# zouyunkai/MedicalSemSeg

Measured on AMD Instinct MI355X. Metric: 96^3 vols/sec fwd+bwd (train), higher is better.
Workload: dtype bf16; 1 GPU; UNet base (MONAI BasicUNet 32-32-64-128-256-32) 1->3cls, 96^3 patches, DiceCE + AdamW, per-GPU batch 2; global_batch=2, parallelism=dp1, grad_sync=none (single rank)

## Files before the change

medicalsemseg_amd/csrc/channel_reduce.h:

```cpp
#pragma once
#include "common.h"

template <typename T> struct ChunkV {
    static constexpr int EPC = DT<T>::EPC;
    float v[EPC];
    MSSEG_DEVFN void load(const T* p) { Chunk<T>::load(p, v); }
    MSSEG_DEVFN void store(T* p) const { Chunk<T>::store(p, v); }
};

static inline bool vec_ok(const void* p, long long ld, int C, int esz) {
    const int epc = 16 / esz;
    return (C % epc) == 0 && (ld % epc) == 0 && (((uintptr_t)p) & 15) == 0;
}

struct RowMap {
    int groups;
    int rows_par;
};
static inline RowMap row_map(int C, int width, int nthr = 256) {
    RowMap m;
    m.groups = ceil_div(C, width);
    if (m.groups > nthr) m.groups = nthr;
    m.rows_par = nthr / m.groups;
    if (m.rows_par < 1) m.rows_par = 1;
    return m;
}

static inline long long reduce_blocks(long long S, int rows_par, int N, int C, int nper) {
    long long blocks = ceil_div_ll(S, (long long)rows_par * 8);
    long long cap = (long long)msseg_num_cus() / (N > 0 ? N : 1);
    if (cap < 1) cap = 1;
    const long long fit = (long long)(((size_t)16 << 20) / ((size_t)N * C * nper * 4));
    if (cap > fit) cap = fit;
    if (blocks > cap) blocks = cap;
    if (blocks < 1) blocks = 1;
    return blocks;
}

constexpr int RED_THREADS = 512;
constexpr int RED_STAGE2 = 16;

template <int W>
MSSEG_DEVFN void block_rows_reduce(float* red, int groups, int rows_par, int g, int rl, bool act) {
    if (act && rl < RED_STAGE2 && rl < rows_par) {
#pragma unroll
        for (int e = 0; e < W; ++e) {
            float a = 0.f, b = 0.f;
            for (int k = rl; k < rows_par; k += RED_STAGE2) {
                a += red[((k * groups + g) * W + e) * 2 + 0];
                b += red[((k * groups + g) * W + e) * 2 + 1];
            }
            red[((rl * groups + g) * W + e) * 2 + 0] = a;
            red[((rl * groups + g) * W + e) * 2 + 1] = b;
        }
    }
    __syncthreads();
}

struct FinalizeArgs {
    const float* ws; int N, nblk, C, nper, mode; float* out; float* dp0; float* dp1; int accumulate;
};
int msseg_channels_finalize_launch(const FinalizeArgs& a, hipStream_t st);
```

medicalsemseg_amd/csrc/head_conv.hip:

```cpp
#include "channel_reduce.h"

namespace {

struct HeadBwdParams {
    const void* dy; long long lddy;
    const float* w;
    const void* x; long long ldx;
    const float* stats; const float* gamma; const float* beta;
    void* da; long long ldda;
    long long S; int C, Cout; float eps, slope;
    int groups, rows_par; long long rows_per_block;
    float* ws;
    int want_dw;
};

struct HeadFinArgs {
    const float* ws; int N, nblk, C, nper, Cout; float* red; float* dbeta; float* dgamma; float* dw; int acc_norm, acc_dw;
};
__global__ __launch_bounds__(256) void head_finalize_kernel(const HeadFinArgs a) {
    __shared__ __attribute__((aligned(16))) float fin[256 * 4 + 64 * 6];
    __shared__ float tot_n[64 * 6];
    const int L = a.C * a.nper;
    for (int o = threadIdx.x; o < L; o += 256) tot_n[o] = 0.f;
    for (int n = 0; n < a.N; ++n) {
        block_rows_sum<256>(a.ws + (long long)n * a.nblk * L, a.nblk, L, fin);
        const float* t = fin + 256 * 4;
        for (int o = threadIdx.x; o < L; o += 256) {
            const int c = o / a.nper, k = o % a.nper;
            if (k < 2) a.red[((long long)n * a.C + c) * 2 + k] = t[o];
            tot_n[o] += t[o];
        }
        __syncthreads();
    }
    for (int o = threadIdx.x; o < L; o += 256) {
        const int c = o / a.nper, k = o % a.nper;
        const float tot = tot_n[o];
        if (k == 0) { if (a.dbeta) a.dbeta[c] = a.acc_norm ? a.dbeta[c] + tot : tot; }
        else if (k == 1) { if (a.dgamma) a.dgamma[c] = a.acc_norm ? a.dgamma[c] + tot : tot; }
        else if (k - 2 < a.Cout && a.dw) a.dw[(k - 2) * a.C + c] = a.acc_dw ? a.dw[(k - 2) * a.C + c] + tot : tot;
    }
}

template <typename T, bool DW>
__global__ __launch_bounds__(RED_THREADS) void head_dgrad_inbwd_kernel(const HeadBwdParams p) {
    constexpr int WD = DT<T>::EPC;
    __shared__ float red[RED_THREADS * 2 * WD];
    const int n = blockIdx.y;
    const int g = threadIdx.x % p.groups, rl = threadIdx.x / p.groups;
    const long long r0 = (long long)blockIdx.x * p.rows_per_block;
    long long r1 = r0 + p.rows_per_block;
    if (r1 > p.S) r1 = p.S;
    const T* xn = (const T*)p.x + (long long)n * p.S * p.ldx;
    const T* dyn = (const T*)p.dy + (long long)n * p.S * p.lddy;
    T* dan = (T*)p.da + (long long)n * p.S * p.ldda;
    for (int gbase = 0; gbase * WD < p.C; gbase += p.groups) {
        const int gg = gbase + g;
        const bool act = gg * WD < p.C;
        float mean[WD], rstd[WD], sc[WD], sh[WD], a0[WD], a1[WD], wv[4][WD];
        float gw[DW ? 4 : 1][WD];
#pragma unroll
        for (int e = 0; e < WD; ++e) {
            const int c = act ? gg * WD + e : 0;
            mean_rstd(p.stats, n, p.C, c, p.S, p.eps, mean[e], rstd[e]);
            sc[e] = rstd[e] * (p.gamma ? p.gamma[c] : 1.f);
            sh[e] = (p.beta ? p.beta[c] : 0.f) - mean[e] * sc[e];
            a0[e] = a1[e] = 0.f;
#pragma unroll
            for (int k = 0; k < 4; ++k) wv[k][e] = k < p.Cout ? (float)(T)p.w[k * p.C + c] : 0.f;
#pragma unroll
            for (int k = 0; k < (DW ? 4 : 1); ++k) gw[k][e] = 0.f;
        }
        if (act && rl < p.rows_par) {
            constexpr int UNR = DW ? 2 : 4;
#pragma unroll UNR
            for (long long r = r0 + rl; r < r1; r += p.rows_par) {
                ChunkV<T> xc, dc, o;
                xc.load(xn + r * p.ldx + gg * WD);
                dc.load(dyn + r * p.lddy);
#pragma unroll
                for (int e = 0; e < WD; ++e) {
                    const float da = head_da<T, WD>(dc.v, wv, e);
                    o.v[e] = da;
                    const float z = xc.v[e] * sc[e] + sh[e];
                    const float dz = z > 0.f ? da : da * p.slope;
                    a0[e] += dz;
                    a1[e] += dz * ((xc.v[e] - mean[e]) * rstd[e]);
                    if constexpr (DW) {
                        const float av = (float)(T)(z > 0.f ? z : z * p.slope);
#pragma unroll
                        for (int k = 0; k < 4; ++k) gw[k][e] += dc.v[k] * av;
                    }
                }
                if (!DW || p.da != nullptr) o.store(dan + r * p.ldda + gg * WD);
            }
        }
        constexpr int NPER = DW ? 6 : 2;
        float* wsb = p.ws + ((long long)n * gridDim.x + blockIdx.x) * p.C * NPER;
#pragma unroll
        for (int round = 0; round < NPER / 2; ++round) {
            __syncthreads();
#pragma unroll
            for (int e = 0; e < WD; ++e) {
                float v0, v1;
                if (round == 0) { v0 = a0[e]; v1 = a1[e]; }
                else { v0 = gw[DW ? 2 * round - 2 : 0][e]; v1 = gw[DW ? 2 * round - 1 : 0][e]; }
                red[(threadIdx.x * WD + e) * 2 + 0] = v0;
                red[(threadIdx.x * WD + e) * 2 + 1] = v1;
            }
            __syncthreads();
            block_rows_reduce<WD>(red, p.groups, p.rows_par, g, rl, act);
            if (act && rl == 0) {
                const int kmax = p.rows_par < RED_STAGE2 ? p.rows_par : RED_STAGE2;
#pragma unroll
                for (int e = 0; e < WD; ++e) {
                    float a = 0.f, b = 0.f;
                    for (int k = 0; k < kmax; ++k) {
                        a += red[((k * p.groups + g) * WD + e) * 2 + 0];
                        b += red[((k * p.groups + g) * WD + e) * 2 + 1];
                    }
                    wsb[(gg * WD + e) * NPER + 2 * round + 0] = a;
                    wsb[(gg * WD + e) * NPER + 2 * round + 1] = b;
                }
            }
        }
    }
}

template <typename T, int COUT>
__global__ __launch_bounds__(256) void conv1x1_head_kernel(const T* __restrict__ x, long long ldx, const float* __restrict__ w,
                                                           const float* __restrict__ bias, T* __restrict__ y, long long ldy,
                                                           long long NV, int Cin) {
    constexpr int WD = DT<T>::EPC;
    __shared__ float wS[COUT * 64];
    for (int i = threadIdx.x; i < COUT * Cin; i += 256) wS[i] = (float)(T)w[i];
    __syncthreads();
    float b[COUT];
#pragma unroll
    for (int c = 0; c < COUT; ++c) b[c] = bias ? bias[c] : 0.f;
    for (long long v = blockIdx.x * 256LL + threadIdx.x; v < NV; v += (long long)gridDim.x * 256) {
        float acc[COUT];
#pragma unroll
        for (int c = 0; c < COUT; ++c) acc[c] = b[c];
        const T* xr = x + v * ldx;
        for (int k0 = 0; k0 < Cin; k0 += 4 * WD) {
            ChunkV<T> xc[4];
#pragma unroll
            for (int j = 0; j < 4; ++j)
                if (k0 + j * WD < Cin) xc[j].load(xr + k0 + j * WD);
#pragma unroll
            for (int j = 0; j < 4; ++j)
                if (k0 + j * WD < Cin) {
#pragma unroll
                    for (int c = 0; c < COUT; ++c)
#pragma unroll
                        for (int e = 0; e < WD; ++e) acc[c] += xc[j].v[e] * wS[c * Cin + k0 + j * WD + e];
                }
        }
        T* yr = y + v * ldy;
#pragma unroll
        for (int c = 0; c < COUT; ++c) DT<T>::st(yr + c, acc[c]);
    }
}

template <typename T, int COUT>
__global__ __launch_bounds__(256) void conv1x1_head_norm_kernel(const T* __restrict__ x, long long ldx,
                                                                const float* __restrict__ stats,
                                                                const float* __restrict__ gamma, const float* __restrict__ beta,
                                                                float slope, float eps, const float* __restrict__ w,
                                                                const float* __restrict__ bias, T* __restrict__ y,
                                                                long long ldy, long long S, int Cin) {
    constexpr int WD = DT<T>::EPC;
    __shared__ float wS[COUT * 64];
    __shared__ float scS[64], shS[64];
    const int n = blockIdx.y;
    for (int i = threadIdx.x; i < COUT * Cin; i += 256) wS[i] = (float)(T)w[i];
    for (int c = threadIdx.x; c < Cin; c += 256) {
        float mean, rstd;
        mean_rstd(stats, n, Cin, c, S, eps, mean, rstd);
        const float sc = rstd * (gamma ? gamma[c] : 1.f);
        scS[c] = sc;
        shS[c] = (beta ? beta[c] : 0.f) - mean * sc;
    }
    __syncthreads();
    float b[COUT];
#pragma unroll
    for (int c = 0; c < COUT; ++c) b[c] = bias ? bias[c] : 0.f;
    const T* xn = x + (long long)n * S * ldx;
    T* yn = y + (long long)n * S * ldy;
    for (long long v = blockIdx.x * 256LL + threadIdx.x; v < S; v += (long long)gridDim.x * 256) {
        float acc[COUT];
#pragma unroll
        for (int c = 0; c < COUT; ++c) acc[c] = b[c];
        const T* xr = xn + v * ldx;
        for (int k0 = 0; k0 < Cin; k0 += 4 * WD) {
            ChunkV<T> xc[4];
#pragma unroll
            for (int j = 0; j < 4; ++j)
                if (k0 + j * WD < Cin) xc[j].load(xr + k0 + j * WD);
#pragma unroll
            for (int j = 0; j < 4; ++j)
                if (k0 + j * WD < Cin) {
#pragma unroll
                    for (int e = 0; e < WD; ++e) {
                        const int k = k0 + j * WD + e;
                        const float z = xc[j].v[e] * scS[k] + shS[k];
                        const float a = (float)(T)(z > 0.f ? z : z * slope);
#pragma unroll
                        for (int c = 0; c < COUT; ++c) acc[c] += a * wS[c * Cin + k];
                    }
                }
        }
        T* yr = yn + v * ldy;
#pragma unroll
        for (int c = 0; c < COUT; ++c) DT<T>::st(yr + c, acc[c]);
    }
}

}

extern "C" {

int msseg_conv3d_k1_head_fwd(const void* x, long long ldx, const float* w, const float* bias, void* y, long long ldy,
                             long long NV, int Cin, int Cout, int dtype, msseg_stream_t stream) {
    if (!x || !w || !y || NV < 1) MSSEG_FAIL(MSSEG_EINVAL, "conv3d_k1_head: bad args");
    const int esz = dtype == MSSEG_F32 ? 4 : 2;
    if (dtype != MSSEG_F32 && dtype != MSSEG_BF16) MSSEG_FAIL(MSSEG_EINVAL, "conv3d_k1_head: bad dtype");
    if (Cout < 1 || Cout > 4 || Cin < 1 || Cin > 64 || !vec_ok(x, ldx, Cin, esz) || ldy < Cout)
        MSSEG_FAIL(MSSEG_EINVAL, "conv3d_k1_head: needs 1 <= Cout <= 4, Cin <= 64 in 16-byte chunks (got %d -> %d)", Cin, Cout);
    const int g = stream_grid(NV);
#define HEAD(T_, C_) hipLaunchKernelGGL((conv1x1_head_kernel<T_, C_>), dim3(g), dim3(256), 0, (hipStream_t)stream, \
                                        (const T_*)x, ldx, w, bias, (T_*)y, ldy, NV, Cin)
#define HEAD_C(T_) do { if (Cout == 1) HEAD(T_, 1); else if (Cout == 2) HEAD(T_, 2); else if (Cout == 3) HEAD(T_, 3); else HEAD(T_, 4); } while (0)
    for_dtype(dtype, [&](auto t) { HEAD_C(typename decltype(t)::type); });
#undef HEAD_C
#undef HEAD
    MSSEG_CHECK_LAUNCH("conv3d_k1_head");
    return MSSEG_OK;
}

int msseg_conv3d_k1_head_bwd_fused(const void* dy, long long lddy, const float* w, void* da, long long ldda, int N,
                                   long long S, int C, int Cout, const void* yraw, long long ldyraw, const float* fwd_stats,
                                   const float* gamma, const float* beta, float slope, float eps, float* red, float* dgamma,
                                   float* dbeta, int accumulate, float* dw, int dw_accumulate, void* scratch,
                                   size_t scratch_bytes, int dtype, msseg_stream_t stream) {
    if (!dy || !w || (!da && !dw) || !yraw || !fwd_stats || !red || N < 1 || S < 1)
        MSSEG_FAIL(MSSEG_EINVAL, "conv3d_k1_head_bwd_fused: bad args");
    if (dtype != MSSEG_F32 && dtype != MSSEG_BF16) MSSEG_FAIL(MSSEG_EINVAL, "conv3d_k1_head_bwd_fused: bad dtype");
    if (int rc = scratch_ok(scratch, scratch_bytes, "conv3d_k1_head_bwd_fused")) return rc;
    const int esz = dtype == MSSEG_F32 ? 4 : 2, epc = 16 / esz;
    if (Cout < 1 || Cout > 4 || C < 1 || C > 64 || !vec_ok(yraw, ldyraw, C, esz) || (da && !vec_ok(da, ldda, C, esz)) ||
        (lddy % epc) || ((uintptr_t)dy & 15))
        MSSEG_FAIL(MSSEG_EINVAL, "conv3d_k1_head_bwd_fused: needs <= 4 classes in 16-byte aligned gradient rows and "
                                 "16-byte channel chunks (C=%d, Cout=%d, lddy=%lld)", C, Cout, lddy);
    HeadBwdParams p{dy, lddy, w, yraw, ldyraw, fwd_stats, gamma, beta, da, ldda, S, C, Cout, eps, slope, 0, 0, 0, nullptr, 0};
    p.ws = (float*)((unsigned char*)scratch + MSSEG_SCRATCH_HEADER_BYTES);
    p.want_dw = dw != nullptr;
    const int nper = dw ? 6 : 2;
    const RowMap m = row_map(C, epc, RED_THREADS);
    p.groups = m.groups; p.rows_par = m.rows_par;
    long long blocks = reduce_blocks(S, m.rows_par, N, C, nper);
    p.rows_per_block = ceil_div_ll(S, blocks);
    blocks = ceil_div_ll(S, p.rows_per_block);
    dim3 grid((unsigned)blocks, N);
    if (dw) {
        for_dtype(dtype, [&](auto t) {
            hipLaunchKernelGGL((head_dgrad_inbwd_kernel<typename decltype(t)::type, true>), grid, dim3(RED_THREADS), 0,
                               (hipStream_t)stream, p);
        });
    } else {
        for_dtype(dtype, [&](auto t) {
            hipLaunchKernelGGL((head_dgrad_inbwd_kernel<typename decltype(t)::type, false>), grid, dim3(RED_THREADS), 0,
                               (hipStream_t)stream, p);
        });
    }
    MSSEG_CHECK_LAUNCH("conv3d_k1_head_dgrad_inbwd");
    HeadFinArgs a{p.ws, N, (int)blocks, C, nper, Cout, red, dbeta, dgamma, dw, accumulate, dw_accumulate};
    hipLaunchKernelGGL(head_finalize_kernel, dim3(1), dim3(256), 0, (hipStream_t)stream, a);
    MSSEG_CHECK_LAUNCH("head_finalize");
    return MSSEG_OK;
}

int msseg_conv3d_k1_head_norm_fwd(const void* x, long long ldx, const float* stats, const float* gamma, const float* beta,
                                  float slope, float eps, const float* w, const float* bias, void* y, long long ldy, int N,
                                  long long S, int Cin, int Cout, int dtype, msseg_stream_t stream) {
    if (!x || !stats || !w || !y || N < 1 || S < 1) MSSEG_FAIL(MSSEG_EINVAL, "conv3d_k1_head_norm: bad args");
    const int esz = dtype == MSSEG_F32 ? 4 : 2;
    if (dtype != MSSEG_F32 && dtype != MSSEG_BF16) MSSEG_FAIL(MSSEG_EINVAL, "conv3d_k1_head_norm: bad dtype");
    if ((gamma == nullptr) != (beta == nullptr)) MSSEG_FAIL(MSSEG_EINVAL, "conv3d_k1_head_norm: gamma/beta go together");
    if (Cout < 1 || Cout > 4 || Cin < 1 || Cin > 64 || !vec_ok(x, ldx, Cin, esz) || ldy < Cout)
        MSSEG_FAIL(MSSEG_EINVAL, "conv3d_k1_head_norm: needs 1 <= Cout <= 4, Cin <= 64 in 16-byte chunks (got %d -> %d)", Cin, Cout);
    long long gx = ceil_div_ll(S, 256);
    const long long cap = (long long)msseg_num_cus() * 16 / N + 1;
    if (gx > cap) gx = cap;
    dim3 grid((unsigned)gx, N);
#define HEADN(T_, C_) hipLaunchKernelGGL((conv1x1_head_norm_kernel<T_, C_>), grid, dim3(256), 0, (hipStream_t)stream, \
                                         (const T_*)x, ldx, stats, gamma, beta, slope, eps, w, bias, (T_*)y, ldy, S, Cin)
#define HEADN_C(T_) do { if (Cout == 1) HEADN(T_, 1); else if (Cout == 2) HEADN(T_, 2); else if (Cout == 3) HEADN(T_, 3); else HEADN(T_, 4); } while (0)
    for_dtype(dtype, [&](auto t) { HEADN_C(typename decltype(t)::type); });
#undef HEADN_C
#undef HEADN
    MSSEG_CHECK_LAUNCH("conv3d_k1_head_norm");
    return MSSEG_OK;
}

}
```

Before: 578.4 vol/s.

## Software-pipeline head backward dW kernel loads and fuse block reduction rounds

```diff
diff --git a/medicalsemseg_amd/csrc/channel_reduce.h b/medicalsemseg_amd/csrc/channel_reduce.h
--- a/medicalsemseg_amd/csrc/channel_reduce.h
+++ b/medicalsemseg_amd/csrc/channel_reduce.h
@@ -57,6 +57,26 @@
     __syncthreads();
 }
 
+template <int NT>
+MSSEG_DEVFN void block_cols_reduce(float* red, int ncols, int rows_par, float* out, int out_cols) {
+    const int slots = rows_par < RED_STAGE2 ? rows_par : RED_STAGE2;
+    for (int item = threadIdx.x; item < slots * ncols; item += NT) {
+        const int s = item / ncols, col = item - s * ncols;
+        float a = 0.f;
+#pragma unroll 8
+        for (int k = s; k < rows_par; k += RED_STAGE2) a += red[k * ncols + col];
+        red[item] = a;
+    }
+    __syncthreads();
+    for (int col = threadIdx.x; col < out_cols; col += NT) {
+        float a = 0.f;
+#pragma unroll
+        for (int k = 0; k < RED_STAGE2; ++k)
+            if (k < slots) a += red[k * ncols + col];
+        out[col] = a;
+    }
+}
+
 struct FinalizeArgs {
     const float* ws; int N, nblk, C, nper, mode; float* out; float* dp0; float* dp1; int accumulate;
 };
diff --git a/medicalsemseg_amd/csrc/head_bwd.h b/medicalsemseg_amd/csrc/head_bwd.h
--- /dev/null
+++ b/medicalsemseg_amd/csrc/head_bwd.h
@@ -0,0 +1,215 @@
+#pragma once
+#include "channel_reduce.h"
+
+struct HeadBwdParams {
+    const void* dy; long long lddy;
+    const float* w;
+    const void* x; long long ldx;
+    const float* stats; const float* gamma; const float* beta;
+    void* da; long long ldda;
+    long long S; int C, Cout; float eps, slope;
+    int groups, rows_par; long long rows_per_block;
+    float* ws;
+    int want_dw;
+};
+
+namespace {
+
+template <typename T> struct ClassRow;
+template <> struct ClassRow<float> {
+    f32x4_t raw;
+    MSSEG_DEVFN void load(const float* p) { raw = *(const f32x4_t*)p; }
+    MSSEG_DEVFN void unpack(float* f) const { f[0] = raw[0]; f[1] = raw[1]; f[2] = raw[2]; f[3] = raw[3]; }
+};
+template <> struct ClassRow<bf16_t> {
+    bf16x4_t raw;
+    MSSEG_DEVFN void load(const bf16_t* p) { raw = *(const bf16x4_t*)p; }
+    MSSEG_DEVFN void unpack(float* f) const { f[0] = (float)raw[0]; f[1] = (float)raw[1]; f[2] = (float)raw[2]; f[3] = (float)raw[3]; }
+};
+
+MSSEG_DEVFN void head_norm_consts(float s, float s2, float gam, float bet, long long S, float eps, float& mean, float& rstd,
+                                  float& sc, float& sh) {
+#pragma clang fp contract(off)
+    const float inv = 1.0f / (float)S;
+    mean = s * inv;
+    float var = __builtin_fmaf(-mean, mean, s2 * inv);
+    var = var > 0.f ? var : 0.f;
+    rstd = rsqrtf(var + eps);
+    sc = rstd * gam;
+    sh = __builtin_fmaf(-mean, sc, bet);
+}
+
+template <typename T, bool STORE, int WD>
+MSSEG_DEVFN void head_row_dw(const u32x4_t& xraw, const ClassRow<T>& draw, const float (*wv)[WD], const float* mean,
+                             const float* rstd, const float* sc, const float* sh, float slope, float* a0, float* a1,
+                             float (*gw)[WD], T* out) {
+#pragma clang fp contract(off)
+    float x[WD], d[4], o[WD];
+    Chunk<T>::unpack(xraw, x);
+    draw.unpack(d);
+#pragma unroll
+    for (int e = 0; e < WD; ++e) {
+        float acc = __builtin_fmaf(d[0], wv[0][e], 0.f);
+#pragma unroll
+        for (int k = 1; k < 4; ++k) acc = __builtin_fmaf(d[k], wv[k][e], acc);
+        const float da = (float)(T)acc;
+        o[e] = da;
+        const float z = __builtin_fmaf(x[e], sc[e], sh[e]);
+        const float dz = z > 0.f ? da : da * slope;
+        a0[e] = a0[e] + dz;
+        const float t = dz * ((x[e] - mean[e]) * rstd[e]);
+        a1[e] = a1[e] + t;
+        const float av = (float)(T)(z > 0.f ? z : z * slope);
+#pragma unroll
+        for (int k = 0; k < 4; ++k) gw[k][e] = __builtin_fmaf(d[k], av, gw[k][e]);
+    }
+    if constexpr (STORE) Chunk<T>::store(out, o);
+}
+
+#ifndef MSSEG_HEAD_DEPTH
+#define MSSEG_HEAD_DEPTH 8
+#endif
+constexpr int HEAD_DEPTH = MSSEG_HEAD_DEPTH;
+
+template <typename T, bool DW, bool STORE>
+__global__ __launch_bounds__(RED_THREADS) void head_dgrad_inbwd_kernel(const HeadBwdParams p) {
+    static_assert(DW || STORE, "the form without dW exists to store da");
+    constexpr int WD = DT<T>::EPC;
+    constexpr int NPER = DW ? 6 : 2;
+    __shared__ float red[RED_THREADS * WD * NPER];
+    const int n = blockIdx.y;
+    const int g = threadIdx.x % p.groups, rl = threadIdx.x / p.groups;
+    const long long r0 = (long long)blockIdx.x * p.rows_per_block;
+    long long r1 = r0 + p.rows_per_block;
+    if (r1 > p.S) r1 = p.S;
+    const T* xn = (const T*)p.x + (long long)n * p.S * p.ldx;
+    const T* dyn = (const T*)p.dy + (long long)n * p.S * p.lddy;
+    T* dan = (T*)p.da + (long long)n * p.S * p.ldda;
+    for (int gbase = 0; gbase * WD < p.C; gbase += p.groups) {
+        const int gg = gbase + g;
+        const bool act = gg * WD < p.C;
+        float mean[WD], rstd[WD], sc[WD], sh[WD], a0[WD], a1[WD], wv[4][WD];
+        float gw[DW ? 4 : 1][WD];
+        constexpr int D = HEAD_DEPTH;
+        constexpr unsigned ES = (unsigned)sizeof(T);
+        const bool live = DW && act && rl < p.rows_par && r0 + rl < r1;
+        const int last = live ? (int)((r1 - 1 - r0 - rl) / p.rows_par) : 0;
+        const char* xb = (const char*)(xn + r0 * p.ldx);
+        const char* db = (const char*)(dyn + r0 * p.lddy);
+        char* ob = STORE ? (char*)(dan + r0 * p.ldda) : nullptr;
+        const unsigned xo = ((unsigned)rl * (unsigned)p.ldx + (unsigned)(gg * WD)) * ES, xs = (unsigned)p.rows_par * (unsigned)p.ldx * ES;
+        const unsigned d0 = (unsigned)rl * (unsigned)p.lddy * ES, ds = (unsigned)p.rows_par * (unsigned)p.lddy * ES;
+        const unsigned oo = ((unsigned)rl * (unsigned)p.ldda + (unsigned)(gg * WD)) * ES, os = (unsigned)p.rows_par * (unsigned)p.ldda * ES;
+        u32x4_t xq[DW ? D : 1];
+        ClassRow<T> dq[DW ? D : 1];
+        if constexpr (DW) {
+            if (live) {
+#pragma unroll
+                for (int i = 0; i < D; ++i) {
+                    const unsigned j = (unsigned)(i < last ? i : last);
+                    xq[i] = ldg16(xb + (xo + j * xs));
+                    dq[i].load((const T*)(db + (d0 + j * ds)));
+                }
+            }
+            const float* gp = p.gamma ? p.gamma : p.stats;
+            const float* bp = p.beta ? p.beta : p.stats;
+            float s1[WD], s2[WD], gv[WD], bv[WD];
+#pragma unroll
+            for (int e = 0; e < WD; ++e) {
+                const int c = act ? gg * WD + e : 0;
+                s1[e] = p.stats[((long long)n * p.C + c) * 2 + 0];
+                s2[e] = p.stats[((long long)n * p.C + c) * 2 + 1];
+                gv[e] = gp[c];
+                bv[e] = bp[c];
+#pragma unroll
+                for (int k = 0; k < 4; ++k) wv[k][e] = p.w[(k < p.Cout ? k : p.Cout - 1) * p.C + c];
+            }
+#pragma unroll
+            for (int e = 0; e < WD; ++e) {
+                head_norm_consts(s1[e], s2[e], p.gamma ? gv[e] : 1.f, p.beta ? bv[e] : 0.f, p.S, p.eps, mean[e], rstd[e], sc[e],
+                                 sh[e]);
+                a0[e] = a1[e] = 0.f;
+#pragma unroll
+                for (int k = 0; k < 4; ++k) {
+                    wv[k][e] = k < p.Cout ? (float)(T)wv[k][e] : 0.f;
+                    gw[k][e] = 0.f;
+                }
+            }
+        } else {
+#pragma unroll
+            for (int e = 0; e < WD; ++e) {
+                const int c = act ? gg * WD + e : 0;
+                mean_rstd(p.stats, n, p.C, c, p.S, p.eps, mean[e], rstd[e]);
+                sc[e] = rstd[e] * (p.gamma ? p.gamma[c] : 1.f);
+                sh[e] = (p.beta ? p.beta[c] : 0.f) - mean[e] * sc[e];
+                a0[e] = a1[e] = 0.f;
+#pragma unroll
+                for (int k = 0; k < 4; ++k) wv[k][e] = k < p.Cout ? (float)(T)p.w[k * p.C + c] : 0.f;
+                gw[0][e] = 0.f;
+            }
+        }
+        if constexpr (DW) {
+            if (live) {
+                int j0 = 0;
+                for (; j0 + D <= last; j0 += D) {
+#pragma unroll
+                    for (int i = 0; i < D; ++i) {
+                        head_row_dw<T, STORE, WD>(xq[i], dq[i], wv, mean, rstd, sc, sh, p.slope, a0, a1, gw,
+                                                  STORE ? (T*)(ob + (oo + (unsigned)(j0 + i) * os)) : nullptr);
+                        const unsigned j = (unsigned)(j0 + i + D < last ? j0 + i + D : last);
+                        xq[i] = ldg16(xb + (xo + j * xs));
+                        dq[i].load((const T*)(db + (d0 + j * ds)));
+                        __builtin_amdgcn_sched_barrier(0);
+                    }
+                }
+#pragma unroll
+                for (int i = 0; i < D; ++i) {
+                    if (j0 + i <= last)
+                        head_row_dw<T, STORE, WD>(xq[i], dq[i], wv, mean, rstd, sc, sh, p.slope, a0, a1, gw,
+                                                  STORE ? (T*)(ob + (oo + (unsigned)(j0 + i) * os)) : nullptr);
+                }
+            }
+        } else {
+            if (act && rl < p.rows_par) {
+#pragma unroll 4
+                for (long long r = r0 + rl; r < r1; r += p.rows_par) {
+                    ChunkV<T> xc, dc, o;
+                    xc.load(xn + r * p.ldx + gg * WD);
+                    dc.load(dyn + r * p.lddy);
+#pragma unroll
+                    for (int e = 0; e < WD; ++e) {
+                        const float da = head_da<T, WD>(dc.v, wv, e);
+                        o.v[e] = da;
+                        const float z = xc.v[e] * sc[e] + sh[e];
+                        const float dz = z > 0.f ? da : da * p.slope;
+                        a0[e] += dz;
+                        a1[e] += dz * ((xc.v[e] - mean[e]) * rstd[e]);
+                    }
+                    o.store(dan + r * p.ldda + gg * WD);
+                }
+            }
+        }
+        const int ncols = p.groups * WD * NPER;
+        __syncthreads();
+        if (rl < p.rows_par) {
+#pragma unroll
+            for (int e = 0; e < WD; ++e) {
+                float* slot = red + (threadIdx.x * WD + e) * NPER;
+                slot[0] = a0[e];
+                slot[1] = a1[e];
+                if constexpr (DW) {
+#pragma unroll
+                    for (int k = 0; k < 4; ++k) slot[2 + k] = gw[k][e];
+                }
+            }
+        }
+        __syncthreads();
+        float* wsb = p.ws + ((long long)n * gridDim.x + blockIdx.x) * p.C * NPER + (long long)gbase * WD * NPER;
+        const int left = (p.C - gbase * WD) * NPER;
+        block_cols_reduce<RED_THREADS>(red, ncols, p.rows_par, wsb, left < ncols ? left : ncols);
+    }
+}
+
+}
+
+void msseg_head_bwd_dw_launch(const HeadBwdParams& p, dim3 grid, int dtype, bool store, hipStream_t st);
diff --git a/medicalsemseg_amd/csrc/head_bwd_dw.hip b/medicalsemseg_amd/csrc/head_bwd_dw.hip
--- /dev/null
+++ b/medicalsemseg_amd/csrc/head_bwd_dw.hip
@@ -0,0 +1,9 @@
+#include "head_bwd.h"
+
+void msseg_head_bwd_dw_launch(const HeadBwdParams& p, dim3 grid, int dtype, bool store, hipStream_t st) {
+    for_dtype(dtype, [&](auto t) {
+        using T = typename decltype(t)::type;
+        if (store) hipLaunchKernelGGL((head_dgrad_inbwd_kernel<T, true, true>), grid, dim3(RED_THREADS), 0, st, p);
+        else hipLaunchKernelGGL((head_dgrad_inbwd_kernel<T, true, false>), grid, dim3(RED_THREADS), 0, st, p);
+    });
+}
diff --git a/medicalsemseg_amd/csrc/head_conv.hip b/medicalsemseg_amd/csrc/head_conv.hip
--- a/medicalsemseg_amd/csrc/head_conv.hip
+++ b/medicalsemseg_amd/csrc/head_conv.hip
@@ -1,18 +1,6 @@
-#include "channel_reduce.h"
+#include "head_bwd.h"
 
 namespace {
-
-struct HeadBwdParams {
-    const void* dy; long long lddy;
-    const float* w;
-    const void* x; long long ldx;
-    const float* stats; const float* gamma; const float* beta;
-    void* da; long long ldda;
-    long long S; int C, Cout; float eps, slope;
-    int groups, rows_par; long long rows_per_block;
-    float* ws;
-    int want_dw;
-};
 
 struct HeadFinArgs {
     const float* ws; int N, nblk, C, nper, Cout; float* red; float* dbeta; float* dgamma; float* dw; int acc_norm, acc_dw;
@@ -38,91 +26,6 @@
         if (k == 0) { if (a.dbeta) a.dbeta[c] = a.acc_norm ? a.dbeta[c] + tot : tot; }
         else if (k == 1) { if (a.dgamma) a.dgamma[c] = a.acc_norm ? a.dgamma[c] + tot : tot; }
         else if (k - 2 < a.Cout && a.dw) a.dw[(k - 2) * a.C + c] = a.acc_dw ? a.dw[(k - 2) * a.C + c] + tot : tot;
-    }
-}
-
-template <typename T, bool DW>
-__global__ __launch_bounds__(RED_THREADS) void head_dgrad_inbwd_kernel(const HeadBwdParams p) {
-    constexpr int WD = DT<T>::EPC;
-    __shared__ float red[RED_THREADS * 2 * WD];
-    const int n = blockIdx.y;
-    const int g = threadIdx.x % p.groups, rl = threadIdx.x / p.groups;
-    const long long r0 = (long long)blockIdx.x * p.rows_per_block;
-    long long r1 = r0 + p.rows_per_block;
-    if (r1 > p.S) r1 = p.S;
-    const T* xn = (const T*)p.x + (long long)n * p.S * p.ldx;
-    const T* dyn = (const T*)p.dy + (long long)n * p.S * p.lddy;
-    T* dan = (T*)p.da + (long long)n * p.S * p.ldda;
-    for (int gbase = 0; gbase * WD < p.C; gbase += p.groups) {
-        const int gg = gbase + g;
-        const bool act = gg * WD < p.C;
-        float mean[WD], rstd[WD], sc[WD], sh[WD], a0[WD], a1[WD], wv[4][WD];
-        float gw[DW ? 4 : 1][WD];
-#pragma unroll
-        for (int e = 0; e < WD; ++e) {
-            const int c = act ? gg * WD + e : 0;
-            mean_rstd(p.stats, n, p.C, c, p.S, p.eps, mean[e], rstd[e]);
-            sc[e] = rstd[e] * (p.gamma ? p.gamma[c] : 1.f);
-            sh[e] = (p.beta ? p.beta[c] : 0.f) - mean[e] * sc[e];
-            a0[e] = a1[e] = 0.f;
-#pragma unroll
-            for (int k = 0; k < 4; ++k) wv[k][e] = k < p.Cout ? (float)(T)p.w[k * p.C + c] : 0.f;
-#pragma unroll
-            for (int k = 0; k < (DW ? 4 : 1); ++k) gw[k][e] = 0.f;
-        }
-        if (act && rl < p.rows_par) {
-            constexpr int UNR = DW ? 2 : 4;
-#pragma unroll UNR
-            for (long long r = r0 + rl; r < r1; r += p.rows_par) {
-                ChunkV<T> xc, dc, o;
-                xc.load(xn + r * p.ldx + gg * WD);
-                dc.load(dyn + r * p.lddy);
-#pragma unroll
-                for (int e = 0; e < WD; ++e) {
-                    const float da = head_da<T, WD>(dc.v, wv, e);
-                    o.v[e] = da;
-                    const float z = xc.v[e] * sc[e] + sh[e];
-                    const float dz = z > 0.f ? da : da * p.slope;
-                    a0[e] += dz;
-                    a1[e] += dz * ((xc.v[e] - mean[e]) * rstd[e]);
-                    if constexpr (DW) {
-                        const float av = (float)(T)(z > 0.f ? z : z * p.slope);
-#pragma unroll
-                        for (int k = 0; k < 4; ++k) gw[k][e] += dc.v[k] * av;
-                    }
-                }
-                if (!DW || p.da != nullptr) o.store(dan + r * p.ldda + gg * WD);
-            }
-        }
-        constexpr int NPER = DW ? 6 : 2;
-        float* wsb = p.ws + ((long long)n * gridDim.x + blockIdx.x) * p.C * NPER;
-#pragma unroll
-        for (int round = 0; round < NPER / 2; ++round) {
-            __syncthreads();
-#pragma unroll
-            for (int e = 0; e < WD; ++e) {
-                float v0, v1;
-                if (round == 0) { v0 = a0[e]; v1 = a1[e]; }
-                else { v0 = gw[DW ? 2 * round - 2 : 0][e]; v1 = gw[DW ? 2 * round - 1 : 0][e]; }
-                red[(threadIdx.x * WD + e) * 2 + 0] = v0;
-                red[(threadIdx.x * WD + e) * 2 + 1] = v1;
-            }
-            __syncthreads();
-            block_rows_reduce<WD>(red, p.groups, p.rows_par, g, rl, act);
-            if (act && rl == 0) {
-                const int kmax = p.rows_par < RED_STAGE2 ? p.rows_par : RED_STAGE2;
-#pragma unroll
-                for (int e = 0; e < WD; ++e) {
-                    float a = 0.f, b = 0.f;
-                    for (int k = 0; k < kmax; ++k) {
-                        a += red[((k * p.groups + g) * WD + e) * 2 + 0];
-                        b += red[((k * p.groups + g) * WD + e) * 2 + 1];
-                    }
-                    wsb[(gg * WD + e) * NPER + 2 * round + 0] = a;
-                    wsb[(gg * WD + e) * NPER + 2 * round + 1] = b;
-                }
-            }
-        }
     }
 }
 
@@ -262,14 +165,15 @@
     p.rows_per_block = ceil_div_ll(S, blocks);
     blocks = ceil_div_ll(S, p.rows_per_block);
     dim3 grid((unsigned)blocks, N);
+    long long ldmax = ldyraw > lddy ? ldyraw : lddy;
+    if (da && ldda > ldmax) ldmax = ldda;
+    if ((p.rows_per_block + 1) * ldmax * esz >= (1LL << 32))
+        MSSEG_FAIL(MSSEG_EINVAL, "conv3d_k1_head_bwd_fused: a block's rows span 4 GB or more (S=%lld, ld=%lld)", S, ldmax);
     if (dw) {
-        for_dtype(dtype, [&](auto t) {
-            hipLaunchKernelGGL((head_dgrad_inbwd_kernel<typename decltype(t)::type, true>), grid, dim3(RED_THREADS), 0,
-                               (hipStream_t)stream, p);
-        });
+        msseg_head_bwd_dw_launch(p, grid, dtype, da != nullptr, (hipStream_t)stream);
     } else {
         for_dtype(dtype, [&](auto t) {
-            hipLaunchKernelGGL((head_dgrad_inbwd_kernel<typename decltype(t)::type, false>), grid, dim3(RED_THREADS), 0,
+            hipLaunchKernelGGL((head_dgrad_inbwd_kernel<typename decltype(t)::type, false, true>), grid, dim3(RED_THREADS), 0,
                                (hipStream_t)stream, p);
         });
     }
```

New measurement: 580.8 vol/s, median of 6. About the same (+0.4%).
